# W298/Surtr

Hardware: AMD Instinct MI355X
Metric: fragments/sec (higher is better)
Workload: dtype f32

## Files before the change

surtr_amd/csrc/clip_core.h:

```cpp
#pragma once
#include <hip/hip_runtime.h>
#include <stdint.h>
#ifndef SURTR_LANES
#define SURTR_LANES 64
#define SURTR_LSH 6
#endif
#ifndef SURTR_WG
#define SURTR_WG 256
#endif
#if SURTR_LANES == 64
#define SURTR_WG_WIDE (4u * SURTR_WG)
#else
#define SURTR_WG_WIDE SURTR_WG
#endif
#define SURTR_NWAVE_WIDE (SURTR_WG_WIDE / SURTR_LANES)
#define SURTR_NWAVE (SURTR_WG / SURTR_LANES)
#ifndef SURTR_DBG
#define SURTR_DBG(...)
#endif

#ifdef SURTR_STAMP
__device__ unsigned long long g_stamp[96];
__device__ unsigned long long g_stamp2[64];
#ifdef SURTR_STAMP_SMALL
// ... 261 lines not shown
template <class Fn>
__device__ void scan_blocks(uint32_t n, uint2* blk, Shared& sh, Fn fn, uint32_t& totC, uint32_t& totW)
{
    const uint32_t nb = (n + SURTR_LANES - 1u) >> SURTR_LSH;
    const uint32_t l = lane_id(), w = wave_id();
    for (uint32_t b = w; b < nb; b += group_waves())
    {
        const uint32_t i = (b << SURTR_LSH) + l;
        uint2 c = make_uint2(0u, 0u);
        if (i < n) c = fn(i);
        uint2 s = wave_incl_scan2(c);
        if (l == SURTR_LANES - 1u) blk[b] = s;
    }
    __syncthreads();
    scan_block_array(nb, blk, sh, totC, totW);
}

template <class I>
__device__ __forceinline__ uint32_t face_next(const I* ring, uint32_t len, uint32_t prev)
{
    if (len <= 4u)
    {
        const uint32_t l1 = len > 1u ? 1u : 0u, l2 = len > 2u ? 2u : 0u, l3 = len > 3u ? 3u : 0u;
        const uint32_t e0 = ring[0], e1 = ring[l1], e2 = ring[l2], e3 = ring[l3];
        const uint32_t last = len == 4u ? e3 : (len == 3u ? e2 : (len == 2u ? e1 : e0));
        if (e0 == prev) return last;
        if (len > 1u && e1 == prev) return e0;
        if (len > 2u && e2 == prev) return e1;
        if (len > 3u && e3 == prev) return e2;
        return last;
// ... 1207 lines not shown
```

surtr_amd/csrc/surtr_hip.hip:

```cpp
#include <algorithm>
#include <cmath>
#include <cstdio>
#include <cstdlib>
#include <cstring>
#include <string>
#include <type_traits>
#include <vector>

#include "surtr_ctx.h"
#include "small_clip.h"
#ifndef SC_RESUME
#define SC_RESUME 1
#endif
#include "literal_clip.h"
#include "wave_clip.h"
#include "prep_sorted.h"

template <uint32_t LV, uint32_t LH>
struct alignas(16) LdsTopoT
{
    static_assert(LV % 16 == 0 && LH % 8 == 0, "clip_image copies 16-byte words into these arrays");
    static constexpr uint32_t kLV = LV, kLH = LH;
    alignas(16) uint16_t loff[LV];
    alignas(16) uint8_t llen[LV];
// ... 1835 lines not shown

__global__ __launch_bounds__(SURTR_LANES) void k_hull_probe(const float* __restrict__ pts, uint32_t n, uint32_t limit, uint32_t* __restrict__ ws,
                                                         float* __restrict__ normals, uint32_t* __restrict__ out )
{
    __shared__ RhLds H;
    __shared__ ArgF slotF[SURTR_NWAVE];
    __shared__ ArgD slotD[SURTR_NWAVE];
    const int rc = rh_build(pts, n, n < limit ? n : limit, (float*)ws, ws + n, H, slotF, slotD);
    if (rc == 0)
        for (uint32_t i = threadIdx.x; i < 3u * H.nLive; i += group_size()) normals[i] = (&H.nrm[0][0])[i];
    if (threadIdx.x == 0) { out[0] = (uint32_t)rc; out[1] = rc == 0 ? H.nLive : 0u; }
}

#ifdef SURTR_STAMP
__device__ unsigned long long g_stamp_faces[8];
#define EAR_T0 const unsigned long long ear_t0 = __builtin_readcyclecounter()
#define EAR_T1 const unsigned long long ear_t1 = __builtin_readcyclecounter()
#define EAR_T2 do { if (lane == 0) { atomicAdd(&g_stamp_faces[2], ear_t1 - ear_t0); atomicAdd(&g_stamp_faces[3], __builtin_readcyclecounter() - ear_t1); atomicAdd(&g_stamp_faces[5], 1ull); } } while (0)
#define FACES_T(name) const unsigned long long name = __builtin_readcyclecounter()
#define FACES_ADD(i, d) do { if (lane_id() == 0) atomicAdd(&g_stamp_faces[i], (unsigned long long)(d)); } while (0)
#else
#define EAR_T0
#define EAR_T1
#define EAR_T2 do { } while (0)
#define FACES_T(name)
#define FACES_ADD(i, d) do { } while (0)
#endif

__device__ __forceinline__ bool on_right(const float* a, const float* b, const float* c, float nx, float ny, float nz)
{
// ... 175 lines not shown
#ifdef SURTR_EAR_SHFL
#define EAR_BCAST(v, i) __shfl(v, i, 64)
#else
#define EAR_BCAST(v, i) lane_bcast(v, (uint32_t)(i))
#endif
    auto bx = [&](int i) { return EAR_BCAST(x, i); };
    auto by = [&](int i) { return EAR_BCAST(y, i); };
    auto bz = [&](int i) { return EAR_BCAST(z, i); };
    const float ax0 = bx(0), ay0 = by(0), az0 = bz(0);
    float nx, ny, nz;
    {
        const float ux = bx(1) - ax0, uy = by(1) - ay0, uz = bz(1) - az0;
        const float wx = bx(2) - ax0, wy = by(2) - ay0, wz = bz(2) - az0;
        nx = uy * wz - uz * wy; ny = uz * wx - ux * wz; nz = ux * wy - uy * wx;
    }
    {
        float sx = 0.f, sy = 0.f, sz = 0.f;
        for (int v = 0; v < N; ++v)
        {
            const int q = v + 1 == N ? 0 : v + 1;
            const float ux = bx(v) - ax0, uy = by(v) - ay0, uz = bz(v) - az0;
            const float wx = bx(q) - ax0, wy = by(q) - ay0, wz = bz(q) - az0;
            sx = sx + (uy * wz - uz * wy); sy = sy + (uz * wx - ux * wz); sz = sz + (ux * wy - uy * wx);
        }
        if (dot3(sx, sy, sz, nx, ny, nz) < 0.f) { nx = -nx; ny = -ny; nz = -nz; }
    }
    int prv = lane == 0 ? N - 1 : lane - 1, nxt = lane + 1 >= N ? 0 : lane + 1;
    auto right_of = [&](float ax, float ay, float az, float bx_, float by_, float bz_, float cx, float cy, float cz) {
        const float ux = bx_ - ax, uy = by_ - ay, uz = bz_ - az;
        const float wx = cx - ax, wy = cy - ay, wz = cz - az;
        const float kx = uy * wz - uz * wy, ky = uz * wx - ux * wz, kz = ux * wy - uy * wx;
        return dot3(kx, ky, kz, nx, ny, nz) > 0.f;
    };
    bool rfx = false;
    {
        const float px_ = __shfl(x, prv, 64), py_ = __shfl(y, prv, 64), pz_ = __shfl(z, prv, 64);
        const float qx = __shfl(x, nxt, 64), qy = __shfl(y, nxt, 64), qz = __shfl(z, nxt, 64);
        rfx = mine && !right_of(px_, py_, pz_, x, y, z, qx, qy, qz);
    }
    EAR_T1;
    int skipped = 0, left = N, cur = 0;
    uint32_t at = 0;
    while (left > 3 && __ballot(rfx) != 0ull)
    {
        const int p = EAR_BCAST(prv, cur), n = EAR_BCAST(nxt, cur);
        const bool cur_reflex = EAR_BCAST((int)rfx, cur) != 0;
        bool ear = !cur_reflex;
        if (ear)
        {
            const float ax = bx(p), ay = by(p), az = bz(p);
            const float cx_ = bx(cur), cy_ = by(cur), cz_ = bz(cur);
            const float ex = bx(n), ey = by(n), ez = bz(n);
            bool inside = false;
            if (mine && rfx && lane != p && lane != n)
            {
                const bool same = (x == ax && y == ay && z == az) || (x == cx_ && y == cy_ && z == cz_);
                if (!same)
                    inside = right_of(ax, ay, az, cx_, cy_, cz_, x, y, z) && right_of(cx_, cy_, cz_, ex, ey, ez, x, y, z) &&
                             right_of(ex, ey, ez, ax, ay, az, x, y, z);
            }
            ear = __ballot(inside) == 0ull;
        }
        if (ear)
        {
            if (lane == 0) { out[at] = (uint32_t)loop[p]; out[at + 1] = (uint32_t)loop[cur]; out[at + 2] = (uint32_t)loop[n]; }
            if (lane == p) nxt = n;
            if (lane == n) prv = p;
            if (lane == cur) nxt = -1;
            const int np = EAR_BCAST(prv, p), nn = EAR_BCAST(nxt, n);
            const float npx = bx(np), npy = by(np), npz = bz(np), nnx = bx(nn), nny = by(nn), nnz = bz(nn);
            const float ppx = bx(p), ppy = by(p), ppz = bz(p), qqx = bx(n), qqy = by(n), qqz = bz(n);
            if (lane == p && rfx) rfx = !right_of(npx, npy, npz, x, y, z, qqx, qqy, qqz);
            if (lane == n && rfx) rfx = !right_of(ppx, ppy, ppz, x, y, z, nnx, nny, nnz);
            at += 3; --left; skipped = 0;
        }
        else if (++skipped > left) { if (lane == 0) out[0] = EAR_STALLED; return 0; }
        cur = n;
    }
    {
        const int p = EAR_BCAST(prv, cur);
        const unsigned long long alive = __ballot(mine && nxt >= 0);
        const unsigned long long below = (1ull << lane) - 1ull, from = ~0ull << cur;
        const uint32_t k = lane >= cur ? (uint32_t)__popcll(alive & from & below) : (uint32_t)__popcll(alive & from) + (uint32_t)__popcll(alive & below);
        if (((alive >> lane) & 1ull) != 0ull && k + 2u < (uint32_t)left)
        {
            uint32_t* o = out + at + 3u * k;
            o[0] = (uint32_t)loop[p]; o[1] = (uint32_t)loop[lane]; o[2] = (uint32_t)loop[nxt];
        }
    }
    EAR_T2;
    return at + 3u * (uint32_t)(left - 2);
}

template <int K, class LP>
__device__ __attribute__((noinline)) static uint32_t ear_clip_face_wave_k(const float* pos, const LP* loop, int N, uint32_t* out)
{
    const int lane = (int)lane_id();
    EAR_T0;
    float x[K], y[K], z[K]; int prv[K], nxt[K]; bool rfx[K], mine[K];
#pragma unroll
    for (int j = 0; j < K; ++j)
    {
// ... 144 lines not shown
            if (((alive[j] >> lane) & 1ull) != 0ull && k + 2u < (uint32_t)left)
            {
                uint32_t* o = out + at + 3u * k;
                o[0] = lp; o[1] = (uint32_t)loop[v]; o[2] = (uint32_t)loop[nxt[j]];
            }
            base += (uint32_t)__popcll(alive[j]);
        }
    }
    EAR_T2;
    return at + 3u * (uint32_t)(left - 2);
}
#endif

struct FacesCompacted { uint32_t at, n; bool full; };
__device__ __attribute__((noinline)) static FacesCompacted faces_compact(uint32_t nfaces, uint2* blk, Shared& sh, const int32_t* faceLo, const int32_t* faceLen,
                                                                         const uint32_t* fcnt, uint32_t* tri, uint32_t* idx, uint32_t* cur_i, uint32_t capI, uint32_t placed_at)
{
    const bool placed = fcnt == nullptr;
    auto src_of = [&](uint32_t fi) -> const uint32_t* {
        const uint32_t lo = (uint32_t)faceLo[fi];
        return placed ? idx + placed_at + 3u * (lo - 2u * fi) : tri + 3u * (size_t)lo;
    };
    auto cntfn = [&](uint32_t fi) -> uint2 {
        if (!placed) return make_uint2(fcnt[fi], 0u);
        return make_uint2(src_of(fi)[0] == EAR_STALLED ? 0u : 3u * ((uint32_t)faceLen[fi] - 2u), 0u);
    };
    uint32_t nidx = 0, dum = 0, at = placed_at;
    scan_blocks(nfaces, blk, sh, cntfn, nidx, dum);
    if (!placed)
    {
        if (threadIdx.x == 0) sh.misc[0] = atomicAdd(cur_i, nidx);
        __syncthreads();
        at = sh.misc[0];
        if ((uint64_t)at + nidx > capI) return FacesCompacted{at, nidx, true};
    }
    uint32_t* const to = placed ? tri : idx + at;
    const uint32_t nb = (nfaces + SURTR_LANES - 1u) >> SURTR_LSH;
    for (uint32_t b = wave_id(); b < nb; b += group_waves())
    {
        const uint32_t fi = (b << SURTR_LSH) + lane_id();
// ... 16 lines not shown
}

__global__ __launch_bounds__(SURTR_WG) __attribute__((amdgpu_waves_per_eu(4, 8))) void k_faces(FragRec* __restrict__ frags, const surtr_counts* __restrict__ counts,
                                                    FaceScratch FS, uint2* __restrict__ blkpool, uint32_t blk_per_wg,
                                                    Arena A, const uint32_t* __restrict__ forder, uint32_t cap_frags,
                                                    uint32_t fan, uint32_t* __restrict__ face_n, uint32_t* __restrict__ face_off,
                                                    int32_t* __restrict__ face_idx, uint32_t* __restrict__ frag_status,
                                                    const uint32_t* __restrict__ take_list, uint32_t* __restrict__ push_list)
{
    __shared__ Shared sh;
#ifndef SURTR_FL_V
#define SURTR_FL_V 1024
#define SURTR_FL_H 4096
#endif
    constexpr uint32_t FL_V = SURTR_FL_V, FL_H = SURTR_FL_H, FL_J = SURTR_FL_H / 2u;
    __shared__ uint16_t f_loff[FL_V]; __shared__ uint16_t f_llen[FL_V]; __shared__ uint16_t f_nbr[FL_H];
    struct IrrLds { uint8_t vis[FL_H]; uint32_t cov[FL_H]; };
    struct JumpLds { uint16_t k0[FL_J], k1[FL_J], x0[FL_J], x1[FL_J], d1[FL_J]; };
    struct EarLds { float pos[3 * FL_V]; uint16_t loop[FL_J]; };
    union FacesLds { IrrLds irr; JumpLds jmp; EarLds ear; };
    static_assert(sizeof(EarLds) <= sizeof(IrrLds), "the ear staging reuses the bytes of the face search");
    static_assert(sizeof(JumpLds) <= sizeof(IrrLds), "the pointer-jumping arrays fit the bytes of the irregular path");
    __shared__ FacesLds FU;
    uint8_t* const f_vis = FU.irr.vis; uint32_t* const f_cov = FU.irr.cov;
    const uint32_t tid = threadIdx.x;
    const uint32_t nf = counts->n_frag;
    int32_t* base = FS.base + (size_t)blockIdx.x * FS.per_wg;
    const uint32_t HF = FS.HF;
    int32_t* keyA = base; int32_t* keyB = base + HF; int32_t* nxA = base + 2 * (size_t)HF; int32_t* nxB = base + 3 * (size_t)HF;
    int32_t* loopbuf = base + 4 * (size_t)HF; int32_t* eartmp = base + 5 * (size_t)HF;
    uint32_t* tri = (uint32_t*)(base + 8 * (size_t)HF);
    uint32_t* fcnt = (uint32_t*)(base + 11 * (size_t)HF);
    uint2* blk = blkpool + (size_t)blockIdx.x * blk_per_wg;
#ifdef SURTR_STAMP
    const unsigned long long wg_t0f = __builtin_readcyclecounter();
#endif
    while (true)
    {
        __syncthreads();
        if (tid == 0)
        {
            if (take_list == nullptr) sh.misc[7] = frag_of_ticket(A, forder, cap_frags, atomicAdd(&A.cursors[CUR_Q_FACES], 1u));
            else { const uint32_t t = atomicAdd(&A.cursors[CUR_Q_FACES2], 1u); sh.misc[7] = t < A.cursors[CUR_FACES2_N] ? take_list[t] : 0xFFFFFFFFu; }
        }
        __syncthreads();
        const uint32_t f = sh.misc[7];
        if (f >= nf) break;
        FragRec fr = frags[f];
        const uint32_t n = fr.mv_n, H = fr.mh_n;
        STAMP_DECL;
#ifdef SURTR_STAMP
        const unsigned long long frag_t0 = __builtin_readcyclecounter();
        if (tid == 0) for (int q = 0; q < 16; ++q) sh.ph[q] = 0;
#endif
        if (H > HF)
        {
            if (tid == 0)
            {
                if (push_list != nullptr) push_list[atomicAdd(&A.cursors[CUR_FACES2_N], 1u)] = f;
                else atomicMax(&A.cursors[CUR_STATUS], (uint32_t)SURTR_E_CAPACITY);
            }
            continue;
        }
        const float* pos = A.pos + 3 * (size_t)fr.mv_off;
        const uint32_t* loff = A.loff + fr.mv_off; const uint32_t* llen = A.llen + fr.mv_off;
        const int32_t* nbr = A.nbr + fr.mh_off;
        const bool topo_lds = n <= FL_V && H <= FL_H && n < 0xFFFFu;
        const bool jump_lds = topo_lds && H <= FL_J;
        if (tid == 0) { sh.flagBad = 0; sh.misc[3] = 0u; sh.misc[4] = 0u; }
        if (topo_lds)
        {
            for (uint32_t v = tid; v < n; v += group_size()) { f_loff[v] = (uint16_t)(loff[v] - fr.mh_off); f_llen[v] = (uint16_t)llen[v]; }
            for (uint32_t e = tid; e < H; e += group_size()) f_nbr[e] = (uint16_t)nbr[e];
        }
        __syncthreads();
        auto gLO = [&](uint32_t v) -> uint32_t { return loff[v] - fr.mh_off; };
        auto gLN = [&](uint32_t v) -> uint32_t { return llen[v]; };
        auto lLO = [&](uint32_t v) -> uint32_t { return f_loff[v]; };
        auto lLN = [&](uint32_t v) -> uint32_t { return f_llen[v]; };
        auto successors = [&](auto LO, auto LN, const auto* NB, auto* NX, auto* KEY, int32_t* copy) {
            typedef typename std::remove_reference<decltype(NX[0])>::type XT;
            bool dup = false;
            for (uint32_t v = tid; v < n; v += group_size())
            {
                const uint32_t lo = LO(v), len = LN(v);
                for (uint32_t s = 0; s < len; ++s)
                {
                    const uint32_t b = (uint32_t)NB[lo + s];
                    for (uint32_t s2 = 0; s2 < s; ++s2) if ((uint32_t)NB[lo + s2] == b) dup = true;
                    const uint32_t lb = LO(b), nbq = LN(b);
                    uint32_t q = 0;
                    while (q < nbq && (uint32_t)NB[lb + q] != v) ++q;
                    const uint32_t sq = (q == 0) ? nbq - 1 : q - 1;
                    NX[lo + s] = (XT)(lb + sq);
                    KEY[lo + s] = (XT)(lo + s);
                    if (copy != nullptr) copy[lo + s] = (int32_t)(lb + sq);
                }
            }
            if (dup) sh.flagBad = 1;
        };
        if (jump_lds) successors(lLO, lLN, f_nbr, FU.jmp.x0, FU.jmp.k0, nxA);
        else if (topo_lds) successors(lLO, lLN, f_nbr, nxA, keyA, (int32_t*)nullptr);
        else successors(gLO, gLN, nbr, nxA, keyA, (int32_t*)nullptr);
        __syncthreads();
        STAMP(60);
        bool irregular = sh.flagBad != 0;
        uint32_t nfaces = 0, lensum = 0;
        int32_t* faceLo = nxB; int32_t* faceLen = keyB;
        bool serial_extract = false;
        int32_t* kc = keyA;
        bool staged = false, failed = false;
        for (int attempt = 0; attempt < 2; ++attempt)
        {
        nfaces = 0; lensum = 0; faceLo = nxB; faceLen = keyB; serial_extract = false; kc = keyA;
        const uint16_t* own16 = nullptr;
        const uint16_t* dist16 = nullptr;
        uint16_t* free16a = nullptr; uint16_t* free16b = nullptr;
        staged = irregular && n <= FL_V && H <= FL_H;
        bool pinched = false;
        if (irregular)
        {
// ... 53 lines not shown
                        const bool canon = slot_of(v, f_nbr[e]) == e;
                        const uint32_t c = f_cov[e];
                        if (canon && (c > e || (c == e) != (f_vis[e] != 0))) mism = true;
                        keyA[e] = (canon && f_vis[e]) ? (int32_t)e : -1;
                    }
                }
                if (mism) sh.flagBad = 2;
                __syncthreads();
                if (sh.flagBad == 2) serial_extract = true;
                __syncthreads();
                faceLo = nxB; faceLen = keyB;
            }
        }
        else if (jump_lds)
        {
            uint16_t* k16 = FU.jmp.k0; uint16_t* kn = FU.jmp.k1; uint16_t* xc = FU.jmp.x0; uint16_t* xn = FU.jmp.x1;
            uint16_t* dc = f_nbr + FL_J; uint16_t* dn = FU.jmp.d1;
            for (uint32_t e = tid; e < H; e += group_size()) dc[e] = 0;
            __syncthreads();
            for (uint32_t span = 1; span < H; span <<= 1)
            {
                for (uint32_t e = tid; e < H; e += group_size())
                {
                    const uint32_t t = xc[e];
                    const uint16_t a = k16[e], b = k16[t];
                    const uint16_t da = dc[e], db = dc[t];
                    kn[e] = a <= b ? a : b;
                    dn[e] = a <= b ? da : (uint16_t)(db + span);
                    xn[e] = xc[t];
                }
                __syncthreads();
                uint16_t* t1 = k16; k16 = kn; kn = t1; t1 = xc; xc = xn; xn = t1; t1 = dc; dc = dn; dn = t1;
            }
// ... 64 lines not shown
                        faceLo[fi] = (int32_t)lo; faceLen[fi] = (int32_t)len;
                        if (len < 3u) sh.misc[3] = 1u;
                    }
                }
                return true;
            };
            auto owners_ranked = [&]() -> bool {
                auto vertex_of = [&](uint32_t e) -> uint32_t {
                    uint32_t lo_v = 0, hi_v = n;
                    while (hi_v - lo_v > 1) { const uint32_t mid = (lo_v + hi_v) >> 1; if (f_loff[mid] <= e) lo_v = mid; else hi_v = mid; }
                    return lo_v;
                };
                bool bad = false;
                for (uint32_t e = tid; e < H; e += group_size())
                {
                    const uint32_t t = (uint32_t)nxA[e], o = own16[e];
                    if (t >= H || own16[t] != o) { bad = true; continue; }
                    const uint32_t want = o == e ? 0u : (t == o ? 1u : (uint32_t)dist16[t] + 1u);
                    if ((uint32_t)dist16[e] != want) bad = true;
                }
                for (uint32_t v = tid; v < n; v += group_size())
                {
                    const uint32_t lo = f_loff[v], len = f_llen[v];
                    for (uint32_t s1 = 1; s1 < len; ++s1)
                        for (uint32_t s2 = 0; s2 < s1; ++s2) if (own16[lo + s1] == own16[lo + s2]) bad = true;
                }
                if (bad) sh.flagBad = 3;
                __syncthreads();
                if (sh.flagBad == 3) { pinched = true; return true; }
                auto ownfn = [&](uint32_t e) -> uint2 {
                    if ((uint32_t)own16[e] != e) return make_uint2(0u, 0u);
                    return make_uint2(1u, (uint32_t)dist16[(uint32_t)nxA[e]] + 1u);
                };
                scan_blocks(H, blk, sh, ownfn, nfaces, lensum);
                if (lensum != H) { pinched = true; return true; }
                uint16_t* lo_of = free16a; uint16_t* len_of = free16b;
                const uint32_t nb = (H + SURTR_LANES - 1u) >> SURTR_LSH;
                for (uint32_t b = wave_id(); b < nb; b += group_waves())
                {
                    const uint32_t e = (b << SURTR_LSH) + lane_id();
                    uint2 c = make_uint2(0u, 0u);
                    if (e < H) c = ownfn(e);
                    const uint2 ex = wave_excl2(c);
                    if (e < H && c.x)
                    {
                        const uint32_t fi = blk[b].x + ex.x, lo = blk[b].y + ex.y;
                        faceLo[fi] = (int32_t)lo; faceLen[fi] = (int32_t)c.y;
                        if (c.y < 3u) sh.misc[3] = 1u;
                        lo_of[e] = (uint16_t)lo; len_of[e] = (uint16_t)c.y;
                    }
                }
                __syncthreads();
                for (uint32_t e = tid; e < H; e += group_size())
                {
                    const uint32_t o = own16[e], d = dist16[e];
                    loopbuf[(uint32_t)lo_of[o] + (d == 0u ? 0u : (uint32_t)len_of[o] - d)] = (int32_t)vertex_of(e);
                }
                return true;
            };
            bool ok;
            if (own16 != nullptr && dist16 != nullptr) ok = owners_ranked();
            else if (own16 != nullptr) ok = owners(lLO, lLN, f_nbr, [&](uint32_t e) { return (uint32_t)own16[e] == e; });
            else if (topo_lds) ok = owners(lLO, lLN, f_nbr, [&](uint32_t e) { return kc[e] == (int32_t)e; });
            else ok = owners(gLO, gLN, nbr, [&](uint32_t e) { return kc[e] == (int32_t)e; });
            if (!ok) { failed = true; break; }
        }
        else
        {
            if (staged) { for (uint32_t e = tid; e < H; e += group_size()) f_vis[e] = 0; }
            else for (uint32_t e = tid; e < H; e += group_size()) keyA[e] = 0;
            __syncthreads();
            auto extract = [&](auto LO, auto LN, auto* NB, auto* visited) {
// ... 44 lines not shown
        __syncthreads();
        if (!pinched) break;
        irregular = true;
        if (tid == 0) { sh.flagBad = 0; sh.misc[3] = 0u; }
        __syncthreads();
        }
        if (failed)
        {
            if (tid == 0)
            {
                frags[f].idx_off = 0; frags[f].idx_n = 0;
                if (frag_status == nullptr || atomicExch(&frag_status[f], (uint32_t)SURTR_E_TOPOLOGY) == 0u) atomicAdd(&A.cursors[CUR_FLAGGED_FRAGS], 1u);
            }
            continue;
        }
        if (face_n != nullptr)
        {
            for (uint32_t fi = tid; fi < nfaces; fi += group_size()) face_off[fi] = (uint32_t)faceLo[fi];
            for (uint32_t e = tid; e < lensum; e += group_size()) face_idx[e] = loopbuf[e];
            if (tid == 0) { face_off[nfaces] = lensum; face_n[0] = nfaces; face_n[1] = lensum; }
        }
        STAMP(62);
        FACES_T(ft_0);
        const bool ear_lds = !fan && n <= FL_V && lensum <= FL_J;
        auto direct = [&]() -> bool { return !fan && SURTR_UNIFORM(sh.misc[3]) == 0u; };
        if (direct() && tid == 0) sh.misc[5] = atomicAdd(&A.cursors[CUR_I], 3u * (lensum - 2u * nfaces));
        __syncthreads();
        if (direct() && (uint64_t)sh.misc[5] + 3u * (lensum - 2u * nfaces) > A.capI) { if (tid == 0) atomicMax(&A.cursors[CUR_STATUS], (uint32_t)SURTR_E_CAPACITY); continue; }
        auto out_of = [&](uint32_t fi, uint32_t lo) -> uint32_t* { return direct() ? A.idx + SURTR_UNIFORM(sh.misc[5]) + 3u * (lo - 2u * fi) : tri + 3u * (size_t)lo; };
        auto count_of = [&](uint32_t fi, uint32_t cnt) {
            if (!direct()) fcnt[fi] = cnt;
            else if (cnt == 0u) sh.misc[4] = 1u;
        };
        if (ear_lds)
        {
            for (uint32_t i = tid; i < 3u * n; i += group_size()) FU.ear.pos[i] = pos[i];
            for (uint32_t e = tid; e < lensum; e += group_size()) FU.ear.loop[e] = (uint16_t)loopbuf[e];
            __syncthreads();
        }
        FACES_T(ft_1);
        FACES_ADD(0, ft_1 - ft_0);
        if (fan)
        {
            for (uint32_t fi = tid; fi < nfaces; fi += group_size())
            {
                const uint32_t lo = (uint32_t)faceLo[fi], len = (uint32_t)faceLen[fi];
                uint32_t* out = tri + 3u * (size_t)lo;
                const int32_t* loop = loopbuf + lo;
                uint32_t at = 0;
                for (uint32_t v = 1; v + 1u < len; ++v) { out[at] = (uint32_t)loop[0]; out[at + 1] = (uint32_t)loop[v]; out[at + 2] = (uint32_t)loop[v + 1]; at += 3u; }
                fcnt[fi] = at;
            }
        }
#if SURTR_LANES == 64
        for (uint32_t f0 = 0; f0 < (fan ? 0u : nfaces); f0 += SURTR_LANES)
        {
            FACES_T(ft_b0);
            const uint32_t fl = f0 + lane_id();
            uint32_t mylo = 0, mylen = 0;
            if (fl < nfaces) { mylo = (uint32_t)faceLo[fl]; mylen = (uint32_t)faceLen[fl]; }
            unsigned long long todo = __ballot(mylen >= 5u && mylen <= SURTR_EAR_WAVE_MAX);
            FACES_ADD(1, __builtin_readcyclecounter() - ft_b0);
            for (uint32_t ord = 0; todo != 0ull; todo &= todo - 1ull, ++ord)
            {
                if (ord % group_waves() != wave_id()) continue;
                const uint32_t src = (uint32_t)__builtin_ctzll(todo);
                const uint32_t lo = lane_bcast(mylo, src), len = lane_bcast(mylen, src);
                uint32_t* const out = out_of(f0 + src, lo);
                uint32_t cnt;
                if (len > 64u) cnt = ear_clip_face_wave_k<SURTR_EAR_WAVE_MAX / 64>(pos, (const int32_t*)loopbuf + lo, (int)len, out);
                else if (ear_lds) cnt = ear_clip_face_wave((const float*)FU.ear.pos, (const uint16_t*)FU.ear.loop + lo, (int)len, out);
                else cnt = ear_clip_face_wave(pos, (const int32_t*)loopbuf + lo, (int)len, out);
                if (lane_id() == 0) count_of(f0 + src, cnt);
            }
        }
        FACES_T(ft_e0);
        __syncthreads();
        FACES_ADD(4, __builtin_readcyclecounter() - ft_e0);
        FACES_ADD(6, __builtin_readcyclecounter() - ft_0);
        STAMP(63);
#endif
        for (uint32_t fi = tid; fi < (fan ? 0u : nfaces); fi += group_size())
        {
            const uint32_t lo = (uint32_t)faceLo[fi], len = (uint32_t)faceLen[fi];
#if SURTR_LANES == 64
            if (len >= 5u && len <= SURTR_EAR_WAVE_MAX) continue;
#endif
            uint32_t* out = out_of(fi, lo);
            uint32_t cnt = 0u;
            if (len >= 3u && len <= 8u)
                cnt = ear_lds ? ear_clip_small((const float*)FU.ear.pos, (const uint16_t*)FU.ear.loop + lo, (int)len, out)
                              : ear_clip_small(pos, (const int32_t*)loopbuf + lo, (int)len, out);
            else if (len > 8u) cnt = ear_clip_face(pos, (const int32_t*)loopbuf + lo, (int)len, eartmp + 3 * (size_t)lo, out);
            count_of(fi, cnt);
#ifdef SURTR_STAMP
            if (len > 64u) { atomicAdd(&g_stamp[66], 1ull); atomicAdd(&g_stamp[67], (unsigned long long)len); }
#endif
        }
        __syncthreads();
        STAMP(64);
        const bool placed = direct();
        uint32_t nidx = placed ? 3u * (lensum - 2u * nfaces) : 0u, idx_at = placed ? sh.misc[5] : 0u;
        if (!placed || sh.misc[4] != 0u)
        {
            const FacesCompacted c = faces_compact(nfaces, blk, sh, faceLo, faceLen, placed ? nullptr : fcnt, tri, A.idx, &A.cursors[CUR_I], A.capI, idx_at);
            if (c.full) { if (tid == 0) atomicMax(&A.cursors[CUR_STATUS], (uint32_t)SURTR_E_CAPACITY); continue; }
            idx_at = c.at; nidx = c.n;
        }
        if (tid == 0) { frags[f].idx_off = idx_at; frags[f].idx_n = nidx; }
        STAMP(65);
#ifdef SURTR_STAMP
        if (tid == 0)
        {
            const unsigned long long d = __builtin_readcyclecounter() - frag_t0;
            int bkt = 0; while ((d >> bkt) > 1 && bkt < 40) ++bkt; bkt = bkt < 12 ? 0 : bkt - 12; if (bkt > 15) bkt = 15;
            atomicAdd(&g_stamp2[32 + bkt], 1ull); atomicAdd(&g_stamp2[51], d);
            for (int q = 0; q < 6; ++q) atomicAdd(&g_stamp2[24 + q], sh.ph[(60 + q) & 15]);
            const unsigned long long old = atomicMax(&g_stamp2[48], d);
            if (d > old) { g_stamp2[49] = n; g_stamp2[50] = H; g_stamp2[55] = nfaces; for (int q = 0; q < 6; ++q) g_stamp2[56 + q] = sh.ph[(60 + q) & 15]; }
        }
// ... 1007 lines not shown
}

static int launch_faces(surtr_ctx* ctx, uint32_t fan, uint32_t* d_face_n, uint32_t* d_face_off, int32_t* d_face_idx)
{
    hipStream_t st = ctx->stream;
    HIPCHK(hipMemsetAsync(ctx->arena.cursors + CUR_Q_FACES, 0, 4, st));
    HIPCHK(hipMemsetAsync(ctx->arena.cursors + CUR_I, 0, 4, st));
    if (!(ctx->last_flags & SURTR_EVT_REFIT))
    {
        HIPCHK(hipMemsetAsync(ctx->arena.cursors + CUR_FLAGGED_FRAGS, 0, 4, st));
        HIPCHK(hipMemsetAsync(ctx->d_frag_status, 0, (size_t)ctx->cap_frags * 4, st));
    }
    PROF_BEGIN(3);
    const bool tiers = ctx->n_wg_faces_big != 0;
    if (tiers) HIPCHK(hipMemsetAsync(ctx->arena.cursors + CUR_FACES2_N, 0, 8, st));
    hipLaunchKernelGGL(k_faces, dim3(std::max(1u, ctx->max_wg_faces)), dim3(SURTR_WG), 0, st, ctx->d_frags, ctx->d_counts, ctx->fs, ctx->d_blk,
                       ctx->blk_per_wg, ctx->arena, ctx->d_forder, ctx->cap_frags, fan, d_face_n, d_face_off, d_face_idx, ctx->d_frag_status,
                       (const uint32_t*)nullptr, tiers ? ctx->d_face_list : (uint32_t*)nullptr);
    if (tiers)
        hipLaunchKernelGGL(k_faces, dim3(ctx->n_wg_faces_big), dim3(SURTR_WG), 0, st, ctx->d_frags, ctx->d_counts, ctx->fs_big, ctx->d_blk_big,
                           ctx->blk_per_wg_big, ctx->arena, ctx->d_forder, ctx->cap_frags, fan, d_face_n, d_face_off, d_face_idx, ctx->d_frag_status,
                           (const uint32_t*)ctx->d_face_list, (uint32_t*)nullptr);
    PROF_END(3);
    hipLaunchKernelGGL(k_out_scan, dim3(1), dim3(SURTR_WG_WIDE), 0, st, ctx->d_frags, ctx->d_scanblk, ctx->d_counts, ctx->arena);
    HIPCHK(hipGetLastError());
    ctx->last_flags |= SURTR_EVT_RENDER; ctx->last_current = false;
    return SURTR_OK;
}

extern "C++" {
int frags_reserve(surtr_ctx* ctx, uint32_t n, uint32_t vmax, uint32_t hmax, uint32_t cvmax, uint32_t chmax, uint64_t MV, uint64_t CV, uint64_t MH, uint64_t CH)
// ... 500 lines not shown
```

Measured before the change: 1.254 million.

## Keep face loops, offsets and positions in LDS; prefetch next fragment ticket

Moves face offset tables, loop vertex indices and small-fragment positions into LDS on the ranked pointer-jumping path, writing global loop buffers only for long faces. Prefetches the next fragment ticket and its header during ear clipping, caches the class counts in LDS, and parities the pointer-jumping buffers so the final result lands in place. Ear clipping reuses the ballot mask for reflex tests and only recomputes neighbour reflexness when it is needed. It also adds an env override for the faces grid size. Several LDS overlays are tied together by offsetof asserts, which makes the aliasing fragile.

```diff
diff --git a/surtr_amd/csrc/clip_core.h b/surtr_amd/csrc/clip_core.h
--- a/surtr_amd/csrc/clip_core.h
+++ b/surtr_amd/csrc/clip_core.h
@@ -299,6 +299,38 @@
     }
     __syncthreads();
     scan_block_array(nb, blk, sh, totC, totW);
+}
+
+template <class Fn>
+__device__ void scan_blocks_lds(uint32_t n, uint2* lblk, Fn fn, uint32_t& totC, uint32_t& totW)
+{
+    const uint32_t nb = (n + SURTR_LANES - 1u) >> SURTR_LSH;
+    const uint32_t l = lane_id(), w = wave_id();
+    for (uint32_t b = w; b < nb; b += group_waves())
+    {
+        const uint32_t i = (b << SURTR_LSH) + l;
+        uint2 c = make_uint2(0u, 0u);
+        if (i < n) c = fn(i);
+        uint2 s = wave_incl_scan2(c);
+        if (l == SURTR_LANES - 1u) lblk[b] = s;
+    }
+    __syncthreads();
+    if (w == 0u)
+    {
+        uint2 carry = make_uint2(0u, 0u);
+        for (uint32_t c0 = 0; c0 < nb; c0 += SURTR_LANES)
+        {
+            const uint32_t i = c0 + l;
+            uint2 x = make_uint2(0u, 0u);
+            if (i < nb) x = lblk[i];
+            const uint2 inc = wave_incl_scan2(x);
+            if (i < nb) lblk[i] = make_uint2(carry.x + inc.x - x.x, carry.y + inc.y - x.y);
+            carry.x += lane_bcast(inc.x, SURTR_LANES - 1u); carry.y += lane_bcast(inc.y, SURTR_LANES - 1u);
+        }
+        if (l == 0u) lblk[nb] = carry;
+    }
+    __syncthreads();
+    totC = lblk[nb].x; totW = lblk[nb].y;
 }
 
 template <class I>
diff --git a/surtr_amd/csrc/surtr_hip.hip b/surtr_amd/csrc/surtr_hip.hip
--- a/surtr_amd/csrc/surtr_hip.hip
+++ b/surtr_amd/csrc/surtr_hip.hip
@@ -1873,6 +1873,8 @@
 
 #ifdef SURTR_STAMP
 __device__ unsigned long long g_stamp_faces[8];
+#endif
+#if defined(SURTR_STAMP) && !defined(SURTR_STAMP_COARSE)
 #define EAR_T0 const unsigned long long ear_t0 = __builtin_readcyclecounter()
 #define EAR_T1 const unsigned long long ear_t1 = __builtin_readcyclecounter()
 #define EAR_T2 do { if (lane == 0) { atomicAdd(&g_stamp_faces[2], ear_t1 - ear_t0); atomicAdd(&g_stamp_faces[3], __builtin_readcyclecounter() - ear_t1); atomicAdd(&g_stamp_faces[5], 1ull); } } while (0)
@@ -2078,38 +2080,33 @@
         const float wx = bx(2) - ax0, wy = by(2) - ay0, wz = bz(2) - az0;
         nx = uy * wz - uz * wy; ny = uz * wx - ux * wz; nz = ux * wy - uy * wx;
     }
-    {
+    int prv = lane == 0 ? N - 1 : lane - 1, nxt = lane + 1 >= N ? 0 : lane + 1;
+    const float px_ = __shfl(x, prv, 64), py_ = __shfl(y, prv, 64), pz_ = __shfl(z, prv, 64);
+    const float qx = __shfl(x, nxt, 64), qy = __shfl(y, nxt, 64), qz = __shfl(z, nxt, 64);
+    {
+        const float ux = x - ax0, uy = y - ay0, uz = z - az0;
+        const float wx = qx - ax0, wy = qy - ay0, wz = qz - az0;
+        const float tx = uy * wz - uz * wy, ty = uz * wx - ux * wz, tz = ux * wy - uy * wx;
         float sx = 0.f, sy = 0.f, sz = 0.f;
-        for (int v = 0; v < N; ++v)
-        {
-            const int q = v + 1 == N ? 0 : v + 1;
-            const float ux = bx(v) - ax0, uy = by(v) - ay0, uz = bz(v) - az0;
-            const float wx = bx(q) - ax0, wy = by(q) - ay0, wz = bz(q) - az0;
-            sx = sx + (uy * wz - uz * wy); sy = sy + (uz * wx - ux * wz); sz = sz + (ux * wy - uy * wx);
-        }
+        for (int v = 0; v < N; ++v) { sx = sx + EAR_BCAST(tx, v); sy = sy + EAR_BCAST(ty, v); sz = sz + EAR_BCAST(tz, v); }
         if (dot3(sx, sy, sz, nx, ny, nz) < 0.f) { nx = -nx; ny = -ny; nz = -nz; }
     }
-    int prv = lane == 0 ? N - 1 : lane - 1, nxt = lane + 1 >= N ? 0 : lane + 1;
     auto right_of = [&](float ax, float ay, float az, float bx_, float by_, float bz_, float cx, float cy, float cz) {
         const float ux = bx_ - ax, uy = by_ - ay, uz = bz_ - az;
         const float wx = cx - ax, wy = cy - ay, wz = cz - az;
         const float kx = uy * wz - uz * wy, ky = uz * wx - ux * wz, kz = ux * wy - uy * wx;
         return dot3(kx, ky, kz, nx, ny, nz) > 0.f;
     };
-    bool rfx = false;
-    {
-        const float px_ = __shfl(x, prv, 64), py_ = __shfl(y, prv, 64), pz_ = __shfl(z, prv, 64);
-        const float qx = __shfl(x, nxt, 64), qy = __shfl(y, nxt, 64), qz = __shfl(z, nxt, 64);
-        rfx = mine && !right_of(px_, py_, pz_, x, y, z, qx, qy, qz);
-    }
+    bool rfx = mine && !right_of(px_, py_, pz_, x, y, z, qx, qy, qz);
     EAR_T1;
     int skipped = 0, left = N, cur = 0;
     uint32_t at = 0;
-    while (left > 3 && __ballot(rfx) != 0ull)
-    {
+    while (left > 3)
+    {
+        const unsigned long long reflex = __ballot(rfx);
+        if (reflex == 0ull) break;
         const int p = EAR_BCAST(prv, cur), n = EAR_BCAST(nxt, cur);
-        const bool cur_reflex = EAR_BCAST((int)rfx, cur) != 0;
-        bool ear = !cur_reflex;
+        bool ear = ((reflex >> cur) & 1ull) == 0ull;
         if (ear)
         {
             const float ax = bx(p), ay = by(p), az = bz(p);
@@ -2127,29 +2124,35 @@
         }
         if (ear)
         {
-            if (lane == 0) { out[at] = (uint32_t)loop[p]; out[at + 1] = (uint32_t)loop[cur]; out[at + 2] = (uint32_t)loop[n]; }
+            const uint32_t o0 = (uint32_t)EAR_BCAST(vid, p), o1 = (uint32_t)EAR_BCAST(vid, cur), o2 = (uint32_t)EAR_BCAST(vid, n);
+            if (lane == 0) { out[at] = o0; out[at + 1] = o1; out[at + 2] = o2; }
             if (lane == p) nxt = n;
             if (lane == n) prv = p;
             if (lane == cur) nxt = -1;
-            const int np = EAR_BCAST(prv, p), nn = EAR_BCAST(nxt, n);
-            const float npx = bx(np), npy = by(np), npz = bz(np), nnx = bx(nn), nny = by(nn), nnz = bz(nn);
-            const float ppx = bx(p), ppy = by(p), ppz = bz(p), qqx = bx(n), qqy = by(n), qqz = bz(n);
-            if (lane == p && rfx) rfx = !right_of(npx, npy, npz, x, y, z, qqx, qqy, qqz);
-            if (lane == n && rfx) rfx = !right_of(ppx, ppy, ppz, x, y, z, nnx, nny, nnz);
+            if ((((reflex >> p) | (reflex >> n)) & 1ull) != 0ull)
+            {
+                const int np = EAR_BCAST(prv, p), nn = EAR_BCAST(nxt, n);
+                const float npx = bx(np), npy = by(np), npz = bz(np), nnx = bx(nn), nny = by(nn), nnz = bz(nn);
+                const float ppx = bx(p), ppy = by(p), ppz = bz(p), qqx = bx(n), qqy = by(n), qqz = bz(n);
+                const bool at_p = lane == p;
+                const float fx = at_p ? npx : ppx, fy = at_p ? npy : ppy, fz = at_p ? npz : ppz;
+                const float gx = at_p ? qqx : nnx, gy = at_p ? qqy : nny, gz = at_p ? qqz : nnz;
+                if ((at_p || lane == n) && rfx) rfx = !right_of(fx, fy, fz, x, y, z, gx, gy, gz);
+            }
             at += 3; --left; skipped = 0;
         }
         else if (++skipped > left) { if (lane == 0) out[0] = EAR_STALLED; return 0; }
         cur = n;
     }
     {
-        const int p = EAR_BCAST(prv, cur);
+        const uint32_t lp = (uint32_t)EAR_BCAST(vid, EAR_BCAST(prv, cur));
         const unsigned long long alive = __ballot(mine && nxt >= 0);
         const unsigned long long below = (1ull << lane) - 1ull, from = ~0ull << cur;
         const uint32_t k = lane >= cur ? (uint32_t)__popcll(alive & from & below) : (uint32_t)__popcll(alive & from) + (uint32_t)__popcll(alive & below);
         if (((alive >> lane) & 1ull) != 0ull && k + 2u < (uint32_t)left)
         {
             uint32_t* o = out + at + 3u * k;
-            o[0] = (uint32_t)loop[p]; o[1] = (uint32_t)loop[lane]; o[2] = (uint32_t)loop[nxt];
+            o[0] = lp; o[1] = (uint32_t)vid; o[2] = (uint32_t)loop[nxt];
         }
     }
     EAR_T2;
@@ -2324,16 +2327,21 @@
 
 struct FacesCompacted { uint32_t at, n; bool full; };
 __device__ __attribute__((noinline)) static FacesCompacted faces_compact(uint32_t nfaces, uint2* blk, Shared& sh, const int32_t* faceLo, const int32_t* faceLen,
+                                                                         const uint16_t* flo16, uint32_t lensum,
                                                                          const uint32_t* fcnt, uint32_t* tri, uint32_t* idx, uint32_t* cur_i, uint32_t capI, uint32_t placed_at)
 {
     const bool placed = fcnt == nullptr;
+    auto lo_of = [&](uint32_t fi) -> uint32_t { return flo16 != nullptr ? (uint32_t)flo16[fi] : (uint32_t)faceLo[fi]; };
+    auto len_of = [&](uint32_t fi) -> uint32_t {
+        return flo16 != nullptr ? (fi + 1u < nfaces ? (uint32_t)flo16[fi + 1u] : lensum) - (uint32_t)flo16[fi] : (uint32_t)faceLen[fi];
+    };
     auto src_of = [&](uint32_t fi) -> const uint32_t* {
-        const uint32_t lo = (uint32_t)faceLo[fi];
+        const uint32_t lo = lo_of(fi);
         return placed ? idx + placed_at + 3u * (lo - 2u * fi) : tri + 3u * (size_t)lo;
     };
     auto cntfn = [&](uint32_t fi) -> uint2 {
         if (!placed) return make_uint2(fcnt[fi], 0u);
-        return make_uint2(src_of(fi)[0] == EAR_STALLED ? 0u : 3u * ((uint32_t)faceLen[fi] - 2u), 0u);
+        return make_uint2(src_of(fi)[0] == EAR_STALLED ? 0u : 3u * (len_of(fi) - 2u), 0u);
     };
     uint32_t nidx = 0, dum = 0, at = placed_at;
     scan_blocks(nfaces, blk, sh, cntfn, nidx, dum);
@@ -2380,14 +2388,30 @@
 #define SURTR_FL_H 4096
 #endif
     constexpr uint32_t FL_V = SURTR_FL_V, FL_H = SURTR_FL_H, FL_J = SURTR_FL_H / 2u;
-    __shared__ uint16_t f_loff[FL_V]; __shared__ uint16_t f_llen[FL_V]; __shared__ uint16_t f_nbr[FL_H];
+    __shared__ uint16_t f_loff[FL_V]; __shared__ uint16_t f_llen[FL_V]; __shared__ __attribute__((aligned(16))) uint16_t f_nbr[FL_H];
     struct IrrLds { uint8_t vis[FL_H]; uint32_t cov[FL_H]; };
     struct JumpLds { uint16_t k0[FL_J], k1[FL_J], x0[FL_J], x1[FL_J], d1[FL_J]; };
-    struct EarLds { float pos[3 * FL_V]; uint16_t loop[FL_J]; };
+    struct EarLds { uint16_t flo[FL_J]; float pos[3 * FL_V]; };
     union FacesLds { IrrLds irr; JumpLds jmp; EarLds ear; };
     static_assert(sizeof(EarLds) <= sizeof(IrrLds), "the ear staging reuses the bytes of the face search");
     static_assert(sizeof(JumpLds) <= sizeof(IrrLds), "the pointer-jumping arrays fit the bytes of the irregular path");
+    static_assert(offsetof(EarLds, flo) == offsetof(JumpLds, k0) && offsetof(EarLds, pos) == offsetof(JumpLds, k1),
+                  "the face table takes the bytes of k0: the ranked route writes it while k1 (the owners) is read");
+    static_assert(offsetof(EarLds, pos) + sizeof(float) * 3 * FL_V <= offsetof(JumpLds, d1),
+                  "the positions take the bytes of k1, x0 and x1, dead after the last pass of the ranked route; d1 is never overlaid");
+    static_assert(2u * FL_J == FL_H, "the loops and the second distance array take the upper half of f_nbr, the successors' copy the lower");
     __shared__ FacesLds FU;
+    uint16_t* const f_loop = f_nbr + FL_J;
+#if (SURTR_FL_H / 2u / SURTR_LANES + 2u) * 8u <= SURTR_FL_H
+    uint2* const f_blk = (uint2*)f_loop;
+#else
+    __shared__ uint2 f_blk[FL_J / SURTR_LANES + 2u];
+#endif
+    constexpr uint32_t FL_PV = (uint32_t)((offsetof(Shared, nzero) - offsetof(Shared, planes)) / (3u * sizeof(float)));
+    static_assert(offsetof(Shared, planes) == 0 && offsetof(Shared, nzero) > offsetof(Shared, zhist), "planes, pmar, hist and zhist lie in a row in front of nzero");
+    float* const f_pos_small = (float*)&sh;
+    constexpr uint32_t LDS_LOOP_MAX = SURTR_LANES == 64 ? 64u : 8u;
+    uint32_t* const f_cls = sh.nzero;
     uint8_t* const f_vis = FU.irr.vis; uint32_t* const f_cov = FU.irr.cov;
     const uint32_t tid = threadIdx.x;
     const uint32_t nf = counts->n_frag;
@@ -2401,18 +2425,38 @@
 #ifdef SURTR_STAMP
     const unsigned long long wg_t0f = __builtin_readcyclecounter();
 #endif
+    constexpr uint32_t TICKET_NONE = 0xFFFFFFFEu;
+    if (take_list == nullptr) for (uint32_t c = tid; c < 16u; c += group_size()) f_cls[c] = A.cursors[CUR_CLS_FRAG + c];
+    if (tid == 0) sh.misc[6] = TICKET_NONE;
+    auto take_ticket = [&]() {
+        uint32_t f = 0xFFFFFFFFu;
+        if (take_list == nullptr)
+        {
+            uint32_t t = atomicAdd(&A.cursors[CUR_Q_FACES], 1u);
+            for (int cls = 15; cls >= 0; --cls)
+            {
+                const uint32_t cnt = f_cls[cls];
+                if (t < cnt) { f = forder[(size_t)cls * cap_frags + t]; break; }
+                t -= cnt;
+            }
+        }
+        else { const uint32_t t = atomicAdd(&A.cursors[CUR_Q_FACES2], 1u); if (t < A.cursors[CUR_FACES2_N]) f = take_list[t]; }
+        sh.misc[6] = f;
+        if (f < nf) { sh.cutmask[0] = frags[f].mv_off; sh.cutmask[1] = frags[f].mv_n; sh.cutmask[2] = frags[f].mh_off; sh.cutmask[3] = frags[f].mh_n; }
+    };
     while (true)
     {
         __syncthreads();
         if (tid == 0)
         {
-            if (take_list == nullptr) sh.misc[7] = frag_of_ticket(A, forder, cap_frags, atomicAdd(&A.cursors[CUR_Q_FACES], 1u));
-            else { const uint32_t t = atomicAdd(&A.cursors[CUR_Q_FACES2], 1u); sh.misc[7] = t < A.cursors[CUR_FACES2_N] ? take_list[t] : 0xFFFFFFFFu; }
+            if (sh.misc[6] == TICKET_NONE) take_ticket();
+            sh.misc[7] = sh.misc[6]; sh.misc[6] = TICKET_NONE;
         }
         __syncthreads();
         const uint32_t f = sh.misc[7];
         if (f >= nf) break;
-        FragRec fr = frags[f];
+        struct { uint32_t mv_off, mv_n, mh_off, mh_n; } fr;
+        fr.mv_off = SURTR_UNIFORM(sh.cutmask[0]); fr.mv_n = SURTR_UNIFORM(sh.cutmask[1]); fr.mh_off = SURTR_UNIFORM(sh.cutmask[2]); fr.mh_n = SURTR_UNIFORM(sh.cutmask[3]);
         const uint32_t n = fr.mv_n, H = fr.mh_n;
         STAMP_DECL;
 #ifdef SURTR_STAMP
@@ -2433,18 +2477,20 @@
         const int32_t* nbr = A.nbr + fr.mh_off;
         const bool topo_lds = n <= FL_V && H <= FL_H && n < 0xFFFFu;
         const bool jump_lds = topo_lds && H <= FL_J;
-        if (tid == 0) { sh.flagBad = 0; sh.misc[3] = 0u; sh.misc[4] = 0u; }
+        if (tid == 0) { sh.flagBad = 0; sh.misc[3] = 0u; sh.misc[4] = 0u; sh.changed = 0u; }
+        const bool pos_small = topo_lds && n <= FL_PV && !fan;
         if (topo_lds)
         {
             for (uint32_t v = tid; v < n; v += group_size()) { f_loff[v] = (uint16_t)(loff[v] - fr.mh_off); f_llen[v] = (uint16_t)llen[v]; }
             for (uint32_t e = tid; e < H; e += group_size()) f_nbr[e] = (uint16_t)nbr[e];
+            if (pos_small) for (uint32_t i = tid; i < 3u * n; i += group_size()) f_pos_small[i] = pos[i];
         }
         __syncthreads();
         auto gLO = [&](uint32_t v) -> uint32_t { return loff[v] - fr.mh_off; };
         auto gLN = [&](uint32_t v) -> uint32_t { return llen[v]; };
         auto lLO = [&](uint32_t v) -> uint32_t { return f_loff[v]; };
         auto lLN = [&](uint32_t v) -> uint32_t { return f_llen[v]; };
-        auto successors = [&](auto LO, auto LN, const auto* NB, auto* NX, auto* KEY, int32_t* copy) {
+        auto successors = [&](auto LO, auto LN, const auto* NB, auto* NX, auto* KEY) {
             typedef typename std::remove_reference<decltype(NX[0])>::type XT;
             bool dup = false;
             for (uint32_t v = tid; v < n; v += group_size())
@@ -2460,17 +2506,20 @@
                     const uint32_t sq = (q == 0) ? nbq - 1 : q - 1;
                     NX[lo + s] = (XT)(lb + sq);
                     KEY[lo + s] = (XT)(lo + s);
-                    if (copy != nullptr) copy[lo + s] = (int32_t)(lb + sq);
                 }
             }
             if (dup) sh.flagBad = 1;
         };
-        if (jump_lds) successors(lLO, lLN, f_nbr, FU.jmp.x0, FU.jmp.k0, nxA);
-        else if (topo_lds) successors(lLO, lLN, f_nbr, nxA, keyA, (int32_t*)nullptr);
-        else successors(gLO, gLN, nbr, nxA, keyA, (int32_t*)nullptr);
+        uint32_t jump_rounds = 0;
+        for (uint32_t span = 1; span < H; span <<= 1) ++jump_rounds;
+        uint16_t* const jk_first = (jump_rounds & 1u) ? FU.jmp.k0 : FU.jmp.k1;
+        if (jump_lds) successors(lLO, lLN, f_nbr, FU.jmp.x0, jk_first);
+        else if (topo_lds) successors(lLO, lLN, f_nbr, nxA, keyA);
+        else successors(gLO, gLN, nbr, nxA, keyA);
         __syncthreads();
         STAMP(60);
         bool irregular = sh.flagBad != 0;
+        bool ranked = false;
         uint32_t nfaces = 0, lensum = 0;
         int32_t* faceLo = nxB; int32_t* faceLen = keyB;
         bool serial_extract = false;
@@ -2554,9 +2603,10 @@
         }
         else if (jump_lds)
         {
-            uint16_t* k16 = FU.jmp.k0; uint16_t* kn = FU.jmp.k1; uint16_t* xc = FU.jmp.x0; uint16_t* xn = FU.jmp.x1;
-            uint16_t* dc = f_nbr + FL_J; uint16_t* dn = FU.jmp.d1;
-            for (uint32_t e = tid; e < H; e += group_size()) dc[e] = 0;
+            const bool odd = (jump_rounds & 1u) != 0u;
+            uint16_t* k16 = jk_first; uint16_t* kn = odd ? FU.jmp.k1 : FU.jmp.k0; uint16_t* xc = FU.jmp.x0; uint16_t* xn = FU.jmp.x1;
+            uint16_t* dc = odd ? f_loop : FU.jmp.d1; uint16_t* dn = odd ? FU.jmp.d1 : f_loop;
+            for (uint32_t e = tid; e < H; e += group_size()) { dc[e] = 0; f_nbr[e] = xc[e]; }
             __syncthreads();
             for (uint32_t span = 1; span < H; span <<= 1)
             {
@@ -2651,7 +2701,7 @@
                 bool bad = false;
                 for (uint32_t e = tid; e < H; e += group_size())
                 {
-                    const uint32_t t = (uint32_t)nxA[e], o = own16[e];
+                    const uint32_t t = f_nbr[e], o = own16[e];
                     if (t >= H || own16[t] != o) { bad = true; continue; }
                     const uint32_t want = o == e ? 0u : (t == o ? 1u : (uint32_t)dist16[t] + 1u);
                     if ((uint32_t)dist16[e] != want) bad = true;
@@ -2667,9 +2717,9 @@
                 if (sh.flagBad == 3) { pinched = true; return true; }
                 auto ownfn = [&](uint32_t e) -> uint2 {
                     if ((uint32_t)own16[e] != e) return make_uint2(0u, 0u);
-                    return make_uint2(1u, (uint32_t)dist16[(uint32_t)nxA[e]] + 1u);
+                    return make_uint2(1u, (uint32_t)dist16[(uint32_t)f_nbr[e]] + 1u);
                 };
-                scan_blocks(H, blk, sh, ownfn, nfaces, lensum);
+                scan_blocks_lds(H, f_blk, ownfn, nfaces, lensum);
                 if (lensum != H) { pinched = true; return true; }
                 uint16_t* lo_of = free16a; uint16_t* len_of = free16b;
                 const uint32_t nb = (H + SURTR_LANES - 1u) >> SURTR_LSH;
@@ -2681,18 +2731,23 @@
                     const uint2 ex = wave_excl2(c);
                     if (e < H && c.x)
                     {
-                        const uint32_t fi = blk[b].x + ex.x, lo = blk[b].y + ex.y;
-                        faceLo[fi] = (int32_t)lo; faceLen[fi] = (int32_t)c.y;
+                        const uint32_t fi = f_blk[b].x + ex.x, lo = f_blk[b].y + ex.y;
                         if (c.y < 3u) sh.misc[3] = 1u;
+                        if (c.y > LDS_LOOP_MAX) sh.changed = 1u;
                         lo_of[e] = (uint16_t)lo; len_of[e] = (uint16_t)c.y;
+                        FU.ear.flo[fi] = (uint16_t)lo;
                     }
                 }
                 __syncthreads();
+                const bool long_face = sh.changed != 0u;
                 for (uint32_t e = tid; e < H; e += group_size())
                 {
                     const uint32_t o = own16[e], d = dist16[e];
-                    loopbuf[(uint32_t)lo_of[o] + (d == 0u ? 0u : (uint32_t)len_of[o] - d)] = (int32_t)vertex_of(e);
+                    const uint32_t at = (uint32_t)lo_of[o] + (d == 0u ? 0u : (uint32_t)len_of[o] - d), v = vertex_of(e);
+                    f_loop[at] = (uint16_t)v;
+                    if (long_face) loopbuf[at] = (int32_t)v;
                 }
+                ranked = true;
                 return true;
             };
             bool ok;
@@ -2767,15 +2822,21 @@
             }
             continue;
         }
+        auto face_lo = [&](uint32_t fi) -> uint32_t { return ranked ? (uint32_t)FU.ear.flo[fi] : (uint32_t)faceLo[fi]; };
+        auto face_len = [&](uint32_t fi, uint32_t lo) -> uint32_t {
+            return ranked ? (fi + 1u < nfaces ? (uint32_t)FU.ear.flo[fi + 1u] : lensum) - lo : (uint32_t)faceLen[fi];
+        };
         if (face_n != nullptr)
         {
-            for (uint32_t fi = tid; fi < nfaces; fi += group_size()) face_off[fi] = (uint32_t)faceLo[fi];
-            for (uint32_t e = tid; e < lensum; e += group_size()) face_idx[e] = loopbuf[e];
+            for (uint32_t fi = tid; fi < nfaces; fi += group_size()) face_off[fi] = face_lo(fi);
+            for (uint32_t e = tid; e < lensum; e += group_size()) face_idx[e] = ranked ? (int32_t)f_loop[e] : loopbuf[e];
             if (tid == 0) { face_off[nfaces] = lensum; face_n[0] = nfaces; face_n[1] = lensum; }
         }
         STAMP(62);
         FACES_T(ft_0);
         const bool ear_lds = !fan && n <= FL_V && lensum <= FL_J;
+        const float* const epos = pos_small ? f_pos_small : FU.ear.pos;
+        if (ear_lds && ranked && !pos_small) for (uint32_t i = tid; i < 3u * n; i += group_size()) FU.ear.pos[i] = pos[i];
         auto direct = [&]() -> bool { return !fan && SURTR_UNIFORM(sh.misc[3]) == 0u; };
         if (direct() && tid == 0) sh.misc[5] = atomicAdd(&A.cursors[CUR_I], 3u * (lensum - 2u * nfaces));
         __syncthreads();
@@ -2785,24 +2846,28 @@
             if (!direct()) fcnt[fi] = cnt;
             else if (cnt == 0u) sh.misc[4] = 1u;
         };
-        if (ear_lds)
-        {
-            for (uint32_t i = tid; i < 3u * n; i += group_size()) FU.ear.pos[i] = pos[i];
-            for (uint32_t e = tid; e < lensum; e += group_size()) FU.ear.loop[e] = (uint16_t)loopbuf[e];
+        if (ear_lds && !ranked)
+        {
+            if (!pos_small) for (uint32_t i = tid; i < 3u * n; i += group_size()) FU.ear.pos[i] = pos[i];
+            for (uint32_t e = tid; e < lensum; e += group_size()) f_loop[e] = (uint16_t)loopbuf[e];
             __syncthreads();
         }
         FACES_T(ft_1);
         FACES_ADD(0, ft_1 - ft_0);
+        if (tid == 0) take_ticket();
         if (fan)
         {
-            for (uint32_t fi = tid; fi < nfaces; fi += group_size())
-            {
-                const uint32_t lo = (uint32_t)faceLo[fi], len = (uint32_t)faceLen[fi];
+            auto fan_face = [&](uint32_t fi, uint32_t lo, uint32_t len, const auto* loop) {
                 uint32_t* out = tri + 3u * (size_t)lo;
-                const int32_t* loop = loopbuf + lo;
                 uint32_t at = 0;
                 for (uint32_t v = 1; v + 1u < len; ++v) { out[at] = (uint32_t)loop[0]; out[at + 1] = (uint32_t)loop[v]; out[at + 2] = (uint32_t)loop[v + 1]; at += 3u; }
                 fcnt[fi] = at;
+            };
+            for (uint32_t fi = tid; fi < nfaces; fi += group_size())
+            {
+                const uint32_t lo = face_lo(fi), len = face_len(fi, lo);
+                if (ranked) fan_face(fi, lo, len, (const uint16_t*)f_loop + lo);
+                else fan_face(fi, lo, len, (const int32_t*)loopbuf + lo);
             }
         }
 #if SURTR_LANES == 64
@@ -2811,7 +2876,7 @@
             FACES_T(ft_b0);
             const uint32_t fl = f0 + lane_id();
             uint32_t mylo = 0, mylen = 0;
-            if (fl < nfaces) { mylo = (uint32_t)faceLo[fl]; mylen = (uint32_t)faceLen[fl]; }
+            if (fl < nfaces) { mylo = face_lo(fl); mylen = face_len(fl, mylo); }
             unsigned long long todo = __ballot(mylen >= 5u && mylen <= SURTR_EAR_WAVE_MAX);
             FACES_ADD(1, __builtin_readcyclecounter() - ft_b0);
             for (uint32_t ord = 0; todo != 0ull; todo &= todo - 1ull, ++ord)
@@ -2822,7 +2887,7 @@
                 uint32_t* const out = out_of(f0 + src, lo);
                 uint32_t cnt;
                 if (len > 64u) cnt = ear_clip_face_wave_k<SURTR_EAR_WAVE_MAX / 64>(pos, (const int32_t*)loopbuf + lo, (int)len, out);
-                else if (ear_lds) cnt = ear_clip_face_wave((const float*)FU.ear.pos, (const uint16_t*)FU.ear.loop + lo, (int)len, out);
+                else if (ear_lds) cnt = ear_clip_face_wave(epos, (const uint16_t*)f_loop + lo, (int)len, out);
                 else cnt = ear_clip_face_wave(pos, (const int32_t*)loopbuf + lo, (int)len, out);
                 if (lane_id() == 0) count_of(f0 + src, cnt);
             }
@@ -2835,14 +2900,14 @@
 #endif
         for (uint32_t fi = tid; fi < (fan ? 0u : nfaces); fi += group_size())
         {
-            const uint32_t lo = (uint32_t)faceLo[fi], len = (uint32_t)faceLen[fi];
+            const uint32_t lo = face_lo(fi), len = face_len(fi, lo);
 #if SURTR_LANES == 64
             if (len >= 5u && len <= SURTR_EAR_WAVE_MAX) continue;
 #endif
             uint32_t* out = out_of(fi, lo);
             uint32_t cnt = 0u;
             if (len >= 3u && len <= 8u)
-                cnt = ear_lds ? ear_clip_small((const float*)FU.ear.pos, (const uint16_t*)FU.ear.loop + lo, (int)len, out)
+                cnt = ear_lds ? ear_clip_small(epos, (const uint16_t*)f_loop + lo, (int)len, out)
                               : ear_clip_small(pos, (const int32_t*)loopbuf + lo, (int)len, out);
             else if (len > 8u) cnt = ear_clip_face(pos, (const int32_t*)loopbuf + lo, (int)len, eartmp + 3 * (size_t)lo, out);
             count_of(fi, cnt);
@@ -2856,7 +2921,8 @@
         uint32_t nidx = placed ? 3u * (lensum - 2u * nfaces) : 0u, idx_at = placed ? sh.misc[5] : 0u;
         if (!placed || sh.misc[4] != 0u)
         {
-            const FacesCompacted c = faces_compact(nfaces, blk, sh, faceLo, faceLen, placed ? nullptr : fcnt, tri, A.idx, &A.cursors[CUR_I], A.capI, idx_at);
+            const FacesCompacted c = faces_compact(nfaces, blk, sh, faceLo, faceLen, ranked ? (const uint16_t*)FU.ear.flo : (const uint16_t*)nullptr, lensum,
+                                                   placed ? nullptr : fcnt, tri, A.idx, &A.cursors[CUR_I], A.capI, idx_at);
             if (c.full) { if (tid == 0) atomicMax(&A.cursors[CUR_STATUS], (uint32_t)SURTR_E_CAPACITY); continue; }
             idx_at = c.at; nidx = c.n;
         }
@@ -3894,7 +3960,9 @@
     PROF_BEGIN(3);
     const bool tiers = ctx->n_wg_faces_big != 0;
     if (tiers) HIPCHK(hipMemsetAsync(ctx->arena.cursors + CUR_FACES2_N, 0, 8, st));
-    hipLaunchKernelGGL(k_faces, dim3(std::max(1u, ctx->max_wg_faces)), dim3(SURTR_WG), 0, st, ctx->d_frags, ctx->d_counts, ctx->fs, ctx->d_blk,
+    uint32_t g_faces = std::max(1u, ctx->max_wg_faces);
+    if (const char* e = getenv("SURTR_FACES_WG")) { const uint32_t v = (uint32_t)atoi(e); if (v > 0 && v <= ctx->n_wg_faces_alloc) g_faces = v; }
+    hipLaunchKernelGGL(k_faces, dim3(g_faces), dim3(SURTR_WG), 0, st, ctx->d_frags, ctx->d_counts, ctx->fs, ctx->d_blk,
                        ctx->blk_per_wg, ctx->arena, ctx->d_forder, ctx->cap_frags, fan, d_face_n, d_face_off, d_face_idx, ctx->d_frag_status,
                        (const uint32_t*)nullptr, tiers ? ctx->d_face_list : (uint32_t*)nullptr);
     if (tiers)
```

Result: no change. 1.264 million, median of 6 (+0.8%).
